# KyleKWKim/LLM-guided-Multimodal-MIL

Measured on AMD Instinct MI355X. Metric: bags/sec fwd+bwd, N=1024 patches D=512, higher is better.
Workload: dtype f32; 1 GPU; 32 bags/GPU x 1024 patches x 512 dims, image-only gated-attention MIL fwd+BCE+bwd+allreduce+Adam (BASELINE config 2; x1 GPUs = 32 bags); bags_per_gpu=32, patches=1024, dim=512, global_bags=32, parallelism=dp1, mode=train (dropout 0.5 on patches + 0.25 before the head, in-kernel masks), accum=1, batches_cycled=4, launch=eager

## Files before the change

### llm-guided-multimodal-mil_amd/csrc/gated_pool.hip

```cpp
#include "mil_common.h"
#include "philox.h"
#include "gate_reduce.h"
#include <type_traits>

#define GF_TM 128
#define GF_BK 32
#define GF_NG 384

typedef __attribute__((address_space(3))) void lds_void;
__device__ __forceinline__ unsigned bitmask1(unsigned m, int b) { return (unsigned)__builtin_amdgcn_sbfe((int)m, b, 1); }
__device__ __forceinline__ float keep_if(float v, unsigned m, int b) {
    return __uint_as_float(__float_as_uint(v) & bitmask1(m, b));
}
template <bool DROP>
__global__ __launch_bounds__(512) void k_gate_fwd(const float* __restrict__ x, const float* __restrict__ Wv,
                                                       const float* __restrict__ bv, const float* __restrict__ Wu,
                                                       const float* __restrict__ bu, const float* __restrict__ wvec,
                                                       const float* __restrict__ battn, float* __restrict__ scores,
                                                       float* __restrict__ gates, int R, int L,
                                                       const uint32_t* __restrict__ xbits, float xscale) {
    __shared__ __attribute__((aligned(16))) float smem[2 * (GF_TM + GF_NG) * 32];
    float* xs = smem;
    float* ws = smem + 2 * GF_TM * 32;
    const int tid = threadIdx.x, lane = tid & 63, wave = tid >> 6;
// ... 1253 lines not shown
    auto xwrite = [&](int i, int buf) {
        f32x4 v = __builtin_bit_cast(f32x4, rx[i]);
        if (DROP) {
            const unsigned mm = rm[i] >> (4 * (xc4 & 7));
#pragma unroll
            for (int e = 0; e < 4; ++e) v[e] = keep_if(v[e], mm, e);
        }
        *reinterpret_cast<f32x4*>(xw + (buf * GB_BKR + 8 * i) * 128) = v;
    };
    auto awrite_v = [&](int i, int buf) {
        const f32x4 v = __builtin_bit_cast(f32x4, rv[i]);
        const f32x4 a = (rds[i] * w4) * __builtin_bit_cast(f32x4, ru[i]);
        const f32x4 t = a * v;
        rt[i] = t;
        *reinterpret_cast<f32x4*>(aw + (buf * GB_BKR + 16 * i) * 128) = a - t * v;
    };
    auto awrite_u = [&](int i, int buf, bool pub) {
        const f32x4 t = rt[i], u = __builtin_bit_cast(f32x4, ru[i]);
        const f32x4 pu = t - t * u;
        *reinterpret_cast<f32x4*>(aw + (buf * GB_BKR + 16 * i) * 128 + 32) = pu;
        if (pub) {
            const f32x4 v = __builtin_bit_cast(f32x4, rv[i]);
            acc_bv += (rds[i] * w4) * u - t * v;
            acc_bu += pu;
            acc_w += (rds[i] * v) * u;
            if (ad4 == 0) acc_ds += rds[i];
        }
    };

    f32x16 acc[2][2];
#pragma unroll
    for (int a = 0; a < 2; ++a)
#pragma unroll
        for (int b = 0; b < 2; ++b)
#pragma unroll
            for (int i = 0; i < 16; ++i) acc[a][b][i] = 0.f;

#pragma unroll
    for (int i = 0; i < 4; ++i) xload(i, rbeg);
#pragma unroll
    for (int i = 0; i < 2; ++i) aload(i, rbeg);
#pragma unroll
    for (int i = 0; i < 4; ++i) xwrite(i, 0);
#pragma unroll
    for (int i = 0; i < 2; ++i) { awrite_v(i, 0); awrite_u(i, 0, jt == 0); }
#pragma unroll
    for (int i = 0; i < 4; ++i) xload(i, rbeg + GB_BKR);
#pragma unroll
    for (int i = 0; i < 2; ++i) aload(i, rbeg + GB_BKR);
    __syncthreads();

    auto slice = [&](int sl, auto buf_c) {
        constexpr int buf = decltype(buf_c)::value;
        const int row2 = rbeg + (sl + 2) * GB_BKR;
        const bool pub = ((sl + 1) % NJ) == jt;
        const float* apb = ap + buf * GB_BKR * 128;
        const float* bpb = bp + buf * GB_BKR * 128;
        float fa[2][2], fb[2][2];
        fa[0][0] = apb[0]; fa[0][1] = apb[64]; fb[0][0] = bpb[0]; fb[0][1] = bpb[64];
#pragma unroll
        for (int ks = 0; ks < GB_BKR / 2; ++ks) {
            const int q = ks & 1;
            acc[0][0] = __builtin_amdgcn_mfma_f32_32x32x2f32(fa[q][0], fb[q][0], acc[0][0], 0, 0, 0);
            __builtin_amdgcn_sched_barrier(0);
            if (ks + 1 < GB_BKR / 2) {
                fa[q ^ 1][0] = apb[(ks + 1) * 256]; fa[q ^ 1][1] = apb[(ks + 1) * 256 + 64];
                fb[q ^ 1][0] = bpb[(ks + 1) * 256]; fb[q ^ 1][1] = bpb[(ks + 1) * 256 + 64];
            }
            __builtin_amdgcn_sched_barrier(0);
            acc[0][1] = __builtin_amdgcn_mfma_f32_32x32x2f32(fa[q][0], fb[q][1], acc[0][1], 0, 0, 0);
            __builtin_amdgcn_sched_barrier(0);
            if (ks >= 1 && ks <= 4) xwrite(ks - 1, buf ^ 1);
            if (ks == 5) awrite_v(0, buf ^ 1);
            if (ks == 6) awrite_u(0, buf ^ 1, pub);
            if (ks == 7) awrite_v(1, buf ^ 1);
            if (ks == 8) awrite_u(1, buf ^ 1, pub);
            __builtin_amdgcn_sched_barrier(0);
            acc[1][0] = __builtin_amdgcn_mfma_f32_32x32x2f32(fa[q][1], fb[q][0], acc[1][0], 0, 0, 0);
            __builtin_amdgcn_sched_barrier(0);
            if (ks >= 1 && ks <= 4) xload(ks - 1, row2);
            if (ks == 6) aload(0, row2);
            if (ks == 8) aload(1, row2);
            __builtin_amdgcn_sched_barrier(0);
            acc[1][1] = __builtin_amdgcn_mfma_f32_32x32x2f32(fa[q][1], fb[q][1], acc[1][1], 0, 0, 0);
            __builtin_amdgcn_sched_barrier(0);
        }
    };
    int sl = 0;
    for (; sl + 1 < nloop; sl += 2) {
        slice(sl, std::integral_constant<int, 0>{});
        __syncthreads();
        slice(sl + 1, std::integral_constant<int, 1>{});
        __syncthreads();
    }
    if (sl < nloop) {
        slice(sl, std::integral_constant<int, 0>{});
        __syncthreads();
    }

    {
        float* tw = smem + wave * (64 * 64);
#pragma unroll
        for (int a = 0; a < 2; ++a)
#pragma unroll
            for (int b = 0; b < 2; ++b)
#pragma unroll
                for (int i = 0; i < 16; ++i) tw[(32 * a + mfma32_row(i, h)) * 64 + 32 * b + r] = acc[a][b][i];
        __syncthreads();
        float* pt = part + ((size_t)s * GF_NG + 128 * m + 64 * wi) * L + j0 + 64 * wj;
        const int c4 = lane & 15, rr = lane >> 4;
        const float* t0 = smem_all + wave * (64 * 64);
        const float* t1 = smem_all + (2 * 2 * GB_BKR * 128) + wave * (64 * 64);
#pragma unroll
        for (int pass = 0; pass < 8; ++pass) {
            const int row = 4 * (pass + 8 * grp) + rr;
            const f32x4 v = *reinterpret_cast<const f32x4*>(t0 + row * 64 + 4 * c4) +
                            *reinterpret_cast<const f32x4*>(t1 + row * 64 + 4 * c4);
            *reinterpret_cast<f32x4*>(pt + (size_t)row * L + 4 * c4) = v;
        }
    }

    {
        float* redf = smem_all;
        const int arow_all = arow + 16 * grp;
        __syncthreads();
#pragma unroll
        for (int e = 0; e < 4; ++e) {
            redf[(arow_all * 3 + 0) * 64 + 4 * ad4 + e] = acc_bv[e];
            redf[(arow_all * 3 + 1) * 64 + 4 * ad4 + e] = acc_bu[e];
            redf[(arow_all * 3 + 2) * 64 + 4 * ad4 + e] = acc_w[e];
        }
        __syncthreads();
        float* pb = pbias + ((size_t)s * NJ + jt) * 4 * 192;
        if (threadIdx.x < 192) {
            const int which = threadIdx.x / 64, d = threadIdx.x % 64;
            float v = 0.f;
#pragma unroll
            for (int g = 0; g < 32; ++g) v += redf[(g * 3 + which) * 64 + d];
            pb[which * 192 + 64 * m + d] = v;
        }
        if (m == 0) {
            __syncthreads();
            redf[threadIdx.x] = acc_ds;
            __syncthreads();
            if (threadIdx.x == 0) {
                float v = 0.f;
                for (int g = 0; g < 512; g += 16) v += redf[g];
                pb[3 * 192] = v;
            }
        }
    }
}

#include "gate_reduce.h"

static inline int split_kg(int R, int L) {
#if defined(GB_NO_KG2)
    return 1;
#endif
    const int NJ = L / 128;
    const int smax = (MIL_NUM_CU) / (3 * NJ);
    return (smax >= 1 && R / smax >= 512) ? 2 : 1;
}
static inline int split_plan(int R, int L, int* KC_out) {
    const int NJ = L / 128;
    int smax = (2 * MIL_NUM_CU / split_kg(R, L)) / (3 * NJ);
    if (smax < 1) smax = 1;
    int kc = ((R + smax - 1) / smax + GB_BKR - 1) / GB_BKR * GB_BKR;
    if (kc < GB_BKR) kc = GB_BKR;
    *KC_out = kc;
    return (R + kc - 1) / kc;
}

extern "C" int mil_abi_version(void) { return 7; }

#define GS_TM 32
#define GS_LS 36
#define GS_THREADS 768
template <bool DROP, int RT>
__global__ __launch_bounds__(GS_THREADS) void k_gate_fwd_r32(const float* __restrict__ x, const float* __restrict__ Wv,
                                                             const float* __restrict__ bv, const float* __restrict__ Wu,
                                                             const float* __restrict__ bu, const float* __restrict__ wvec,
                                                             const float* __restrict__ battn, float* __restrict__ scores,
                                                             float* __restrict__ gates, int R, int L,
                                                             const uint32_t* __restrict__ xbits, float xscale,
                                                             const int32_t* __restrict__ rows_dev) {
    constexpr int TM = GS_TM * RT;
    if (rows_dev != nullptr && (int)(blockIdx.x * TM) >= __builtin_amdgcn_readfirstlane(rows_dev[0])) return;
    __shared__ __attribute__((aligned(16))) float smem[2 * (TM + GF_NG) * GS_LS];
    float* xs = smem;
    float* ws = smem + 2 * TM * GS_LS;
    const int tid = threadIdx.x, lane = tid & 63, wave = tid >> 6;
    const int c = wave >> 1, isu = wave & 1;
    const int r = lane & 31, h = lane >> 5;
    const int row0 = blockIdx.x * TM;
    const float* wsrc[4];
    int wdst[4];
#pragma unroll
    for (int i = 0; i < 4; ++i) {
        const int id = tid + GS_THREADS * i, wrow = id >> 3, ch = id & 7;
        wsrc[i] = (wrow < 192 ? Wv + (size_t)wrow * L : Wu + (size_t)(wrow - 192) * L) + 4 * ch;
        wdst[i] = wrow * GS_LS + 4 * ch;
    }
    const int xrow = (tid % (256 * RT)) >> 3, xch = tid & 7;
    const float* xsrc = x + (size_t)min(row0 + xrow, R - 1) * L + 4 * xch;
    const uint32_t* msrc = DROP ? xbits + (size_t)min(row0 + xrow, R - 1) * (L / 32) : nullptr;
    const int xdst = xrow * GS_LS + 4 * xch;
    f32x4 wreg[2][4], xreg[2];
    unsigned mreg[2] = {0, 0};
    auto gload = [&](int set, int k0) {
#pragma unroll
        for (int i = 0; i < 4; ++i) wreg[set][i] = *reinterpret_cast<const f32x4*>(wsrc[i] + k0);
        xreg[set] = *reinterpret_cast<const f32x4*>(xsrc + k0);
        if (DROP) mreg[set] = msrc[k0 >> 5];
    };
    auto swrite = [&](int set, int buf) {
#pragma unroll
        for (int i = 0; i < 4; ++i) *reinterpret_cast<f32x4*>(ws + buf * GF_NG * GS_LS + wdst[i]) = wreg[set][i];
        if (tid < 256 * RT) {
            f32x4 v = xreg[set];
            if (DROP) {
                const unsigned m = mreg[set] >> (4 * xch);
#pragma unroll
                for (int e = 0; e < 4; ++e) v[e] = keep_if(v[e], m, e) * xscale;
            }
            *reinterpret_cast<f32x4*>(xs + buf * TM * GS_LS + xdst) = v;
        }
    };
    f32x16 acc[RT];
#pragma unroll
    for (int q = 0; q < RT; ++q)
#pragma unroll
        for (int i = 0; i < 16; ++i) acc[q][i] = 0.f;
    const int nslice = L / GF_BK;
    gload(0, 0);
    swrite(0, 0);
    gload(1, min(1, nslice - 1) * GF_BK);
    gload(0, min(2, nslice - 1) * GF_BK);
    __syncthreads();
    auto iteration = [&](int s, int set) {
        const int buf = s & 1;
        const float* xa = xs + buf * TM * GS_LS + r * GS_LS + 4 * h;
        const float* wb = ws + buf * GF_NG * GS_LS + (192 * isu + 32 * c + r) * GS_LS + 4 * h;
        f32x4 fa[RT][4], fb[4];
#pragma unroll
        for (int t = 0; t < 4; ++t) {
#pragma unroll
            for (int q = 0; q < RT; ++q) fa[q][t] = *reinterpret_cast<const f32x4*>(xa + q * GS_TM * GS_LS + 8 * t);
            fb[t] = *reinterpret_cast<const f32x4*>(wb + 8 * t);
        }
        swrite(set, buf ^ 1);
        gload(set, min(s + 3, nslice - 1) * GF_BK);
        __builtin_amdgcn_sched_barrier(0);
#pragma unroll
        for (int t = 0; t < 4; ++t)
#pragma unroll
            for (int jj = 0; jj < 4; ++jj)
#pragma unroll
                for (int q = 0; q < RT; ++q) acc[q] = __builtin_amdgcn_mfma_f32_32x32x2f32(fa[q][t][jj], fb[t][jj], acc[q], 0, 0, 0);
        __syncthreads();
    };
    for (int s = 0; s < nslice; s += 2) {
        iteration(s, 1);
        if (s + 1 < nslice) iteration(s + 1, 0);
    }
    const int d = 32 * c + r;
    float* uex = smem;
    float* sred = smem + 6 * 32 * 33;
#pragma unroll
    for (int q = 0; q < RT; ++q) {
        float gv[16];
        if (q > 0) __syncthreads();
        if (isu) {
            const float bud = bu[d];
#pragma unroll
            for (int i = 0; i < 16; ++i) {
                gv[i] = fast_sigmoid(acc[q][i] + bud);
                uex[(c * 32 + mfma32_row(i, h)) * 33 + r] = gv[i];
            }
        } else {
            const float bvd = bv[d];
#pragma unroll
            for (int i = 0; i < 16; ++i) gv[i] = fast_tanh(acc[q][i] + bvd);
        }
        if (gates != nullptr) {
#pragma unroll
            for (int i = 0; i < 16; ++i) {
                const int gr = row0 + GS_TM * q + mfma32_row(i, h);
                if (gr < R) gates[(size_t)gr * GF_NG + 192 * isu + d] = gv[i];
            }
        }
        __syncthreads();
        if (!isu) {
            const float wd = wvec[d];
#pragma unroll
            for (int i = 0; i < 16; ++i) {
                const int lr = mfma32_row(i, h);
                const float part = half_allsum(wd * gv[i] * uex[(c * 32 + lr) * 33 + r]);
                if (r == 0) sred[c * GS_TM + lr] = part;
            }
        }
        __syncthreads();
        if (tid < GS_TM && row0 + GS_TM * q + tid < R) {
            float sc = battn[0];
#pragma unroll
            for (int cc = 0; cc < 6; ++cc) sc += sred[cc * GS_TM + tid];
            scores[row0 + GS_TM * q + tid] = sc;
// ... 198 lines not shown
        g.offset_dev = offset_dev;
        return gate_scores_fwd_impl(x, Wv, bv, Wu, bu, w, b, scores, gates, R, L, MIL_GATE_D, nullptr, xscale, &g, stream, nullptr,
                                    nullptr, rows_dev, tmap, Wp);
    }
    return gate_scores_fwd_impl(x, Wv, bv, Wu, bu, w, b, scores, gates, R, L, MIL_GATE_D, xbits, xscale, nullptr, stream, nullptr,
                                nullptr, rows_dev, tmap, Wp);
}

int gate_fwd_with_pool(const float* x, const float* Wv, const float* bv, const float* Wu, const float* bu, const float* w,
                       const float* b, float* scores, float* gates, int R, int L, int draw, uint32_t* xbits, float xscale,
                       uint32_t* mbits, float mscale, int B, uint64_t seed, uint64_t mseed, uint64_t offset,
                       const int32_t* offset_dev, const int32_t* tile_map, int T, float* partials, const float* Wf, float* hrow,
                       int* fused, void* stream, const uint16_t* Wp) {
    GateFwdPool pl{};
    pl.tile_map = tile_map;
    pl.partials = partials;
    pl.T = T;
    pl.Wf = Wf;
    pl.hrow = hrow;
    pl.mbits = draw ? nullptr : mbits;
    pl.mscale = mscale;
    if (draw) {
        if (!xbits || !mbits || (L % 64) != 0 || B <= 0) return MIL_EINVAL;
        GateFwdGen g{};
        g.xbits_out = xbits;
        g.mbits_out = mbits;
        g.B = B;
        g.seed_lo = (uint32_t)seed;
        g.seed_hi = (uint32_t)(seed >> 32);
        g.mseed_lo = (uint32_t)mseed;
        g.mseed_hi = (uint32_t)(mseed >> 32);
        g.offset = offset;
        g.offset_dev = offset_dev;
        return gate_scores_fwd_impl(x, Wv, bv, Wu, bu, w, b, scores, gates, R, L, MIL_GATE_D, nullptr, xscale, &g, stream, &pl, fused,
                                    nullptr, nullptr, Wp);
    }
    return gate_scores_fwd_impl(x, Wv, bv, Wu, bu, w, b, scores, gates, R, L, MIL_GATE_D, xbits, xscale, nullptr, stream, &pl, fused,
                                nullptr, nullptr, Wp);
}

static int launch_pool_partial(const float* x, const float* scores, const int32_t* tile_map, int T, int L,
                               float* partials, const float* Wf, int C, float* hrow, hipStream_t st,
                               const uint32_t* xbits = nullptr, float xscale = 1.0f, const uint32_t* mbits = nullptr,
                               float mscale = 1.0f) {
    if (T <= 0) return MIL_OK;
    const bool nt = (size_t)T * MIL_POOL_TILE * L * sizeof(float) > MIL_STREAM_BYTES;
#define POOL_LAUNCH(NQ_) do { \
        if (nt) hipLaunchKernelGGL((k_pool_partial<NQ_, true>), dim3(T), dim3(256), 0, st, x, scores, tile_map, partials, L, Wf, C, hrow, xbits, xscale, mbits, mscale); \
        else hipLaunchKernelGGL((k_pool_partial<NQ_, false>), dim3(T), dim3(256), 0, st, x, scores, tile_map, partials, L, Wf, C, hrow, xbits, xscale, mbits, mscale); } while (0)
    switch (L / 256) {
        case 1: POOL_LAUNCH(1); break;
        case 2: POOL_LAUNCH(2); break;
        case 3: POOL_LAUNCH(3); break;
        default: POOL_LAUNCH(4); break;
    }
#undef POOL_LAUNCH
    MIL_CHECK_LAUNCH();
    return MIL_OK;
}

__global__ __launch_bounds__(256) void k_build_tile_map(const int32_t* __restrict__ bag_len, int B, int32_t* __restrict__ tile_map,
                                                        int32_t* __restrict__ bag_tile_off, int32_t* __restrict__ rows_out,
                                                        int T_cap) {
    build_tile_map_block(bag_len, B, tile_map, bag_tile_off, rows_out, T_cap);
}

extern "C" int mil_build_tile_map(const int32_t* bag_len, int B, int32_t* tile_map, int32_t* bag_tile_off, int32_t* rows_out,
                                  int T_cap, void* stream) {
    if (!bag_len || !tile_map || !bag_tile_off || !rows_out || B <= 0 || B > 1024 || T_cap < 0) return MIL_EINVAL;
    hipLaunchKernelGGL(k_build_tile_map, dim3(1), dim3(256), 0, (hipStream_t)stream, bag_len, B, tile_map, bag_tile_off, rows_out,
                       T_cap);
    MIL_CHECK_LAUNCH();
    return MIL_OK;
}

extern "C" int mil_attn_pool_partial_h(const float* x, const float* scores, const int32_t* tile_map, int T, int L,
                                       float* partials, const float* Wf, int C, float* hrow, const uint32_t* xbits,
                                       float xscale, const uint32_t* mbits, float mscale, void* stream) {
    if (!x || !scores || !tile_map || !partials || !Wf || !hrow) return MIL_EINVAL;
    if (L <= 0 || (L % 256) != 0 || L > 1024 || T < 0 || C <= 0 || C > 4) return MIL_EINVAL;
    return launch_pool_partial(x, scores, tile_map, T, L, partials, Wf, C, hrow, (hipStream_t)stream, xbits, xscale, mbits,
                               mscale);
}

extern "C" int mil_attn_pool_bwd_from_h(const float* scores, const float* lse, const float* hrow, const float* dz,
                                        const float* cdot, const int32_t* tile_map, int T, int C, float* ds, void* stream) {
    if (!scores || !lse || !hrow || !dz || !cdot || !tile_map || !ds || T < 0 || C <= 0 || C > 4) return MIL_EINVAL;
    if (T == 0) return MIL_OK;
    hipLaunchKernelGGL(k_pool_ds_from_h, dim3((T + 7) / 8), dim3(256), 0, (hipStream_t)stream, scores, lse, hrow, dz, cdot,
                       tile_map, T, C, ds);
    MIL_CHECK_LAUNCH();
    return MIL_OK;
}

extern "C" int mil_attn_pool_partial(const float* x, const float* scores, const int32_t* tile_map, int T, int L,
                                     float* partials, const uint32_t* xbits, float xscale, void* stream) {
    if (!x || !scores || !tile_map || !partials) return MIL_EINVAL;
    if (L <= 0 || (L % 256) != 0 || L > 1024 || T < 0) return MIL_EINVAL;
    return launch_pool_partial(x, scores, tile_map, T, L, partials, nullptr, 0, nullptr, (hipStream_t)stream, xbits, xscale);
}

extern "C" int mil_attn_pool_fwd(const float* x, const float* scores, const int32_t* tile_map,
                                 const int32_t* bag_tile_off, int T, int B, int L, float* partials, float* M,
                                 float* lse, const uint32_t* xbits, float xscale, void* stream) {
    if (!x || !scores || !tile_map || !bag_tile_off || !partials || !M || !lse) return MIL_EINVAL;
    if (L <= 0 || (L % 256) != 0 || L > 1024 || B < 0 || T < 0) return MIL_EINVAL;
    hipStream_t st = (hipStream_t)stream;
    const int rc = launch_pool_partial(x, scores, tile_map, T, L, partials, nullptr, 0, nullptr, st, xbits, xscale);
    if (rc != MIL_OK) return rc;
    if (B > 0) {
        hipLaunchKernelGGL(k_pool_merge, dim3(B, L / 128), dim3(256), 0, st, partials, bag_tile_off, M, lse, L, T);
        MIL_CHECK_LAUNCH();
    }
    return MIL_OK;
}

extern "C" int mil_attn_pool_bwd(const float* x, const float* scores, const float* lse, const float* dM,
                                 const float* cdot, const int32_t* tile_map, int T, int L, float* ds, float* dx,
                                 const uint32_t* xbits, float xscale, void* stream) {
    if (!x || !scores || !lse || !dM || !cdot || !tile_map || !ds) return MIL_EINVAL;
    if (L <= 0 || (L % 256) != 0 || L > 1024 || T < 0) return MIL_EINVAL;
    if (T == 0) return MIL_OK;
    hipStream_t st = (hipStream_t)stream;
    switch (L / 256) {
        case 1: hipLaunchKernelGGL(k_pool_bwd_ds<1>, dim3(T), dim3(256), 0, st, x, scores, lse, dM, cdot, tile_map, ds, dx, L, xbits, xscale); break;
        case 2: hipLaunchKernelGGL(k_pool_bwd_ds<2>, dim3(T), dim3(256), 0, st, x, scores, lse, dM, cdot, tile_map, ds, dx, L, xbits, xscale); break;
        case 3: hipLaunchKernelGGL(k_pool_bwd_ds<3>, dim3(T), dim3(256), 0, st, x, scores, lse, dM, cdot, tile_map, ds, dx, L, xbits, xscale); break;
        default: hipLaunchKernelGGL(k_pool_bwd_ds<4>, dim3(T), dim3(256), 0, st, x, scores, lse, dM, cdot, tile_map, ds, dx, L, xbits, xscale); break;
    }
    MIL_CHECK_LAUNCH();
    return MIL_OK;
}

template <bool XB16>
static void launch_gate_bwd_dw(const void* x, const float* gates, const float* ds, const float* w, float* part, float* pbias,
                               int R, int L, int kc, int NJ, int S, const uint32_t* xbits, hipStream_t st,
                               const int32_t* rows_dev = nullptr) {
    const dim3 grid(S * 3 * NJ);
    if (split_kg(R, L) == 2) {
        if (xbits) hipLaunchKernelGGL((k_gate_bwd_dw<XB16, 2, true>), grid, dim3(512), 0, st, x, gates, ds, w, part, pbias, R, L, kc, NJ, xbits, rows_dev);
        else hipLaunchKernelGGL((k_gate_bwd_dw<XB16, 2, false>), grid, dim3(512), 0, st, x, gates, ds, w, part, pbias, R, L, kc, NJ, xbits, rows_dev);
    } else {
        if (xbits) hipLaunchKernelGGL((k_gate_bwd_dw<XB16, 1, true>), grid, dim3(256), 0, st, x, gates, ds, w, part, pbias, R, L, kc, NJ, xbits, rows_dev);
        else hipLaunchKernelGGL((k_gate_bwd_dw<XB16, 1, false>), grid, dim3(256), 0, st, x, gates, ds, w, part, pbias, R, L, kc, NJ, xbits, rows_dev);
    }
}

static inline bool use_dw2(int R, int L) {
#if defined(GB_NO_DW2)
    return false;
#endif
    return split_kg(R, L) == 2 && (long long)R * L < (1ll << 29);
}
static inline size_t gate_bwd_ws_floats(int S, int L) { return (size_t)S * GF_NG * L + (size_t)S * (L / 128) * 4 * 192; }

extern "C" size_t mil_gate_bwd_workspace_floats(int R, int L) {
    if (R <= 0 || L <= 0 || (L % 128) != 0) return 0;
    int kc;
    const int S = split_plan(R, L, &kc);
    return gate_bwd_ws_floats(S, L);
}

static int gate_bwd_partials_impl(const float* x, const float* gates, const float* ds, const float* w, int R, int L,
                                  int D, float* workspace, size_t workspace_floats, const uint32_t* xbits,
                                  const int32_t* rows_dev, void* stream) {
    if (!x || !gates || !ds || !w || !workspace) return MIL_EINVAL;
    if (D != MIL_GATE_D || L <= 0 || (L % 128) != 0 || R <= 0) return MIL_EINVAL;
    int kc;
    const int S = split_plan(R, L, &kc);
    if (workspace_floats < gate_bwd_ws_floats(S, L)) return MIL_ENOSPC;
    const int NJ = L / 128;
    if (use_dw2(R, L)) {
        float* pb = workspace + (size_t)S * GF_NG * L;
        if (xbits)
            hipLaunchKernelGGL(k_gate_bwd_dw2<true>, dim3(S * 3 * NJ), dim3(512), 0, (hipStream_t)stream, x, gates, ds, w, workspace, pb,
                               R, L, kc, NJ, xbits, rows_dev);
        else
            hipLaunchKernelGGL(k_gate_bwd_dw2<false>, dim3(S * 3 * NJ), dim3(512), 0, (hipStream_t)stream, x, gates, ds, w, workspace, pb,
                               R, L, kc, NJ, xbits, rows_dev);
        MIL_CHECK_LAUNCH();
        return MIL_OK;
    }
    launch_gate_bwd_dw<false>((const void*)x, gates, ds, w, workspace, workspace + (size_t)S * GF_NG * L, R, L, kc, NJ, S, xbits,
                              (hipStream_t)stream, rows_dev);
    MIL_CHECK_LAUNCH();
    return MIL_OK;
}

extern "C" int mil_gate_bwd_partials(const float* x, const float* gates, const float* ds, const float* w, int R, int L,
                                     int D, float* workspace, size_t workspace_floats, const uint32_t* xbits,
                                     void* stream) {
    return gate_bwd_partials_impl(x, gates, ds, w, R, L, D, workspace, workspace_floats, xbits, nullptr, stream);
}
extern "C" int mil_gate_bwd_partials_rows(const float* x, const float* gates, const float* ds, const float* w, int R, int L,
                                          int D, float* workspace, size_t workspace_floats, const uint32_t* xbits,
                                          const int32_t* rows_dev, void* stream) {
    return gate_bwd_partials_impl(x, gates, ds, w, R, L, D, workspace, workspace_floats, xbits, rows_dev, stream);
}

extern "C" int mil_gate_bwd_reduce(const float* workspace, int R, int L, float* dWv, float* dbv, float* dWu, float* dbu,
                                   float* dw, float* db, int accumulate, float xscale, void* stream) {
    if (!workspace || !dWv || !dbv || !dWu || !dbu || !dw || !db) return MIL_EINVAL;
    if (L <= 0 || (L % 128) != 0 || R <= 0) return MIL_EINVAL;
    int kc;
    const int S = split_plan(R, L, &kc);
    const int nthreads = GF_NG * (L / 4) + GR_NB * (3 * 192 + 1);
    hipLaunchKernelGGL(k_gate_bwd_reduce, dim3((nthreads + 255) / 256), dim3(256), 0, (hipStream_t)stream, workspace,
                       workspace + (size_t)S * GF_NG * L, S, use_dw2(R, L) ? S * (L / 128) : S, L, dWv, dbv, dWu, dbu, dw, db,
                       accumulate, xscale);
    MIL_CHECK_LAUNCH();
    return MIL_OK;
}

extern "C" int mil_gate_bwd_params_head(const float* x, const float* gates, const float* ds, const float* w, int R, int L,
                                        int D, float* workspace, size_t workspace_floats, float* dWv, float* dbv,
                                        float* dWu, float* dbu, float* dw, float* db, int accumulate, const float* dz,
                                        const float* M, float* dWf, float* dbf, int B, int C, const float* loss_bag,
                                        float* loss_out, const uint32_t* xbits, float xscale, void* stream) {
    if (!dWv || !dbv || !dWu || !dbu || !dw || !db || !dz || !M || !dWf || !dbf) return MIL_EINVAL;
    if (B <= 0 || C <= 0 || C > 32 || (loss_bag && !loss_out)) return MIL_EINVAL;
    const int rc = mil_gate_bwd_partials(x, gates, ds, w, R, L, D, workspace, workspace_floats, xbits, stream);
    if (rc != MIL_OK) return rc;
    int kc;
    const int S = split_plan(R, L, &kc);
    const int nthreads = GF_NG * (L / 4) + GR_NB * (3 * 192 + 1);
    const int nred = (nthreads + 255) / 256, nhead = C * ((L + 63) / 64) + 1;
    const HeadBwdArgs head{dz, M, dWf, dbf, loss_bag, loss_out, B, L, C, accumulate};
    hipLaunchKernelGGL(k_gate_bwd_reduce, dim3(nred + nhead), dim3(256), 0, (hipStream_t)stream, workspace,
                       workspace + (size_t)S * GF_NG * L, S, use_dw2(R, L) ? S * (L / 128) : S, L, dWv, dbv, dWu, dbu, dw, db,
                       accumulate, xbits ? xscale : 1.0f, nred, head);
    MIL_CHECK_LAUNCH();
    return MIL_OK;
}

extern "C" int mil_gate_bwd_reduce_head(const float* workspace, int R, int L, float* dWv, float* dbv, float* dWu, float* dbu,
                                        float* dw, float* db, int accumulate, float xscale, const float* dz, const float* M,
                                        float* dWf, float* dbf, int B, int C, const float* loss_bag, float* loss_out,
                                        void* stream) {
    if (!workspace || !dWv || !dbv || !dWu || !dbu || !dw || !db || !dz || !M || !dWf || !dbf) return MIL_EINVAL;
    if (L <= 0 || (L % 128) != 0 || R <= 0 || B <= 0 || C <= 0 || C > 32 || (loss_bag && !loss_out)) return MIL_EINVAL;
    int kc;
    const int S = split_plan(R, L, &kc);
    const int nthreads = GF_NG * (L / 4) + GR_NB * (3 * 192 + 1);
    const int nred = (nthreads + 255) / 256, nhead = C * ((L + 63) / 64) + 1;
    const HeadBwdArgs head{dz, M, dWf, dbf, loss_bag, loss_out, B, L, C, accumulate};
    hipLaunchKernelGGL(k_gate_bwd_reduce, dim3(nred + nhead), dim3(256), 0, (hipStream_t)stream, workspace,
                       workspace + (size_t)S * GF_NG * L, S, use_dw2(R, L) ? S * (L / 128) : S, L, dWv, dbv, dWu, dbu, dw, db,
                       accumulate, xscale, nred, head);
    MIL_CHECK_LAUNCH();
    return MIL_OK;
}

int gate_bwd_reduce_head_adam_impl(const float* workspace, int R, int L, float* dWv, float* dbv, float* dWu, float* dbu,
                                   float* dw, float* db, int accumulate, float xscale, const float* dz, const float* M,
                                   float* dWf, float* dbf, int B, int C, const float* loss_bag, float* loss_out,
                                   float* param_flat, const float* grad_flat, size_t n_param, float* exp_avg,
                                   float* exp_avg_sq, int step, const int* step_dev, float lr, const float* lr_dev, float beta1,
                                   float beta2, float eps, float weight_decay, float grad_scale, void* stream, int* done = nullptr,
                                   uint16_t* Wp = nullptr);

extern "C" int mil_gate_bwd_reduce_head_adam(const float* workspace, int R, int L, float* dWv, float* dbv, float* dWu,
                                             float* dbu, float* dw, float* db, int accumulate, float xscale, const float* dz,
                                             const float* M, float* dWf, float* dbf, int B, int C, const float* loss_bag,
                                             float* loss_out, float* param_flat, const float* grad_flat, size_t n_param,
                                             float* exp_avg, float* exp_avg_sq, int step, float lr, float beta1, float beta2,
                                             float eps, float weight_decay, float grad_scale, void* stream) {
    return gate_bwd_reduce_head_adam_impl(workspace, R, L, dWv, dbv, dWu, dbu, dw, db, accumulate, xscale, dz, M, dWf, dbf, B, C,
                                          loss_bag, loss_out, param_flat, grad_flat, n_param, exp_avg, exp_avg_sq, step, nullptr,
                                          lr, nullptr, beta1, beta2, eps, weight_decay, grad_scale, stream);
}

int gate_bwd_reduce_head_adam_impl(const float* workspace, int R, int L, float* dWv, float* dbv, float* dWu, float* dbu,
                                   float* dw, float* db, int accumulate, float xscale, const float* dz, const float* M,
                                   float* dWf, float* dbf, int B, int C, const float* loss_bag, float* loss_out,
                                   float* param_flat, const float* grad_flat, size_t n_param, float* exp_avg,
                                   float* exp_avg_sq, int step, const int* step_dev, float lr, const float* lr_dev, float beta1,
                                   float beta2, float eps, float weight_decay, float grad_scale, void* stream, int* done,
                                   uint16_t* Wp) {
    if (!workspace || !dWv || !dbv || !dWu || !dbu || !dw || !db || !dz || !M || !dWf || !dbf) return MIL_EINVAL;
    if (!param_flat || !grad_flat || !exp_avg || !exp_avg_sq || (step_dev == nullptr && step < 1)) return MIL_EINVAL;
    if (step_dev != nullptr) step = 1;
    if (L <= 0 || (L % 128) != 0 || R <= 0 || B <= 0 || C <= 0 || C > 32 || (loss_bag && !loss_out)) return MIL_EINVAL;
    const float* outs[8] = {dWv, dbv, dWu, dbu, dw, db, dWf, dbf};
    const size_t lens[8] = {(size_t)192 * L, 192, (size_t)192 * L, 192, 192, 1, (size_t)C * L, (size_t)C};
    for (int i = 0; i < 8; ++i)
        if (outs[i] < grad_flat || outs[i] + lens[i] > grad_flat + n_param) return MIL_EINVAL;
    if (((dWv - grad_flat) | (dWu - grad_flat)) & 3) return MIL_EINVAL;
    if ((reinterpret_cast<uintptr_t>(param_flat) | reinterpret_cast<uintptr_t>(grad_flat) | reinterpret_cast<uintptr_t>(exp_avg) |
         reinterpret_cast<uintptr_t>(exp_avg_sq)) & 15)
        return MIL_EINVAL;
    int kc;
    const int S = split_plan(R, L, &kc);
    const int nthreads = GF_NG * (L / 4) + GR_NB * (3 * 192 + 1);
    const int nred = (nthreads + 255) / 256, nhead = C * ((L + 63) / 64) + 1;
    const HeadBwdArgs head{dz, M, dWf, dbf, loss_bag, loss_out, B, L, C, accumulate};
    const double bc1 = 1.0 - pow((double)beta1, (double)step);
    const double bc2 = 1.0 - pow((double)beta2, (double)step);
    const AdamFuse ad{param_flat, grad_flat, exp_avg, exp_avg_sq, (float)bc1, beta1, beta2, eps, weight_decay, grad_scale,
                      (float)sqrt(bc2), step_dev, lr, lr_dev, step_dev ? done : nullptr};
    hipLaunchKernelGGL(k_gate_bwd_reduce, dim3(nred + nhead), dim3(256), 0, (hipStream_t)stream, workspace,
                       workspace + (size_t)S * GF_NG * L, S, use_dw2(R, L) ? S * (L / 128) : S, L, dWv, dbv, dWu, dbu, dw, db,
                       accumulate, xscale, nred, head, ad, nullptr, nullptr, (unsigned short*)Wp);
    MIL_CHECK_LAUNCH();
    return MIL_OK;
}

__global__ __launch_bounds__(256) void k_gate_pieces(const float* __restrict__ Wv, const float* __restrict__ Wu,
                                                     unsigned short* __restrict__ Wp, int L) {
    const int L4 = L / 4;
    const int idx = blockIdx.x * 256 + threadIdx.x;
    if (idx >= GF_NG * L4) return;
    const int n = idx / L4, k = 4 * (idx % L4);
    const float* src = (n < MIL_GATE_D ? Wv + (size_t)n * L : Wu + (size_t)(n - MIL_GATE_D) * L) + k;
    gp_store4(Wp, n, k, *reinterpret_cast<const f32x4*>(src));
}

extern "C" int mil_gate_pieces(const float* Wv, const float* Wu, uint16_t* Wp, int L, void* stream) {
    if (!Wv || !Wu || !Wp || L <= 0 || (L % 32) != 0) return MIL_EINVAL;
    if ((reinterpret_cast<uintptr_t>(Wv) | reinterpret_cast<uintptr_t>(Wu) | reinterpret_cast<uintptr_t>(Wp)) & 15) return MIL_EINVAL;
    hipLaunchKernelGGL(k_gate_pieces, dim3((GF_NG * (L / 4) + 255) / 256), dim3(256), 0, (hipStream_t)stream, Wv, Wu,
                       (unsigned short*)Wp, L);
    MIL_CHECK_LAUNCH();
    return MIL_OK;
}

extern "C" int mil_gate_bwd_params(const float* x, const float* gates, const float* ds, const float* w, int R, int L,
// ... 290 lines not shown
```

Before: 153,900 bags/s.

## Add split-bf16 MFMA weight-gradient kernel for gated attention backward

Adds a new weight-gradient kernel for the gate backward pass. It splits each f32 operand into three bf16 pieces and accumulates six cross products with 32x32x16 bf16 MFMA, standing in for the previous dW path. It double-buffers LDS staging and interleaves global loads and LDS writes with the MFMA steps. It also remaps block IDs across XCDs and folds the bias and w-vector reductions into the same kernel. The kernel is on by default, with an environment variable to turn it off, and it trades some precision (roughly f32 via 3xbf16) for matrix-core throughput.

```diff
diff --git a/llm-guided-multimodal-mil_amd/csrc/gated_pool.hip b/llm-guided-multimodal-mil_amd/csrc/gated_pool.hip
--- a/llm-guided-multimodal-mil_amd/csrc/gated_pool.hip
+++ b/llm-guided-multimodal-mil_amd/csrc/gated_pool.hip
@@ -1429,7 +1429,249 @@
     }
 }
 
-#include "gate_reduce.h"
+typedef float dwp_f32x2 __attribute__((ext_vector_type(2)));
+typedef __bf16 dwp_bf16x2 __attribute__((ext_vector_type(2)));
+#define DWP_IMG_BYTES (3 * 2 * 128 * 16)
+#define DWP_PIECE_BYTES (2 * 128 * 16)
+
+__device__ __forceinline__ void dwp_split8(const float (&v)[8], u32x4_t (&out)[3]) {
+#pragma unroll
+    for (int i = 0; i < 4; ++i) {
+        const dwp_f32x2 v2 = {v[2 * i], v[2 * i + 1]};
+        const dwp_bf16x2 p0 = __builtin_convertvector(v2, dwp_bf16x2);
+        dwp_f32x2 r1 = v2 - __builtin_convertvector(p0, dwp_f32x2);
+        r1[0] = __builtin_isfinite(r1[0]) ? r1[0] : 0.f;
+        r1[1] = __builtin_isfinite(r1[1]) ? r1[1] : 0.f;
+        const dwp_bf16x2 p1 = __builtin_convertvector(r1, dwp_bf16x2);
+        const dwp_f32x2 r2 = r1 - __builtin_convertvector(p1, dwp_f32x2);
+        const dwp_bf16x2 p2 = __builtin_convertvector(r2, dwp_bf16x2);
+        out[0][i] = __builtin_bit_cast(unsigned, p0);
+        out[1][i] = __builtin_bit_cast(unsigned, p1);
+        out[2][i] = __builtin_bit_cast(unsigned, p2);
+    }
+}
+__device__ __forceinline__ float dwp_keep_lane(float v, uint64_t lanemask) {
+    float o;
+    asm("v_cndmask_b32_e64 %0, 0, %1, %2" : "=v"(o) : "v"(v), "s"(lanemask));
+    return o;
+}
+
+template <bool DROP>
+__global__ __launch_bounds__(512) void k_gate_bwd_dw2p(const float* __restrict__ x, const float* __restrict__ gates,
+                                                       const float* __restrict__ ds, const float* __restrict__ wvec,
+                                                       float* __restrict__ part, float* __restrict__ pbias, int R, int L,
+                                                       int KC, int NJ, const uint32_t* __restrict__ xbits,
+                                                       const int32_t* __restrict__ rows_dev) {
+    __shared__ __attribute__((aligned(16))) float smem_all[2 * 2 * 2 * GB_BKR * 128];
+    if (rows_dev != nullptr) R = min(R, __builtin_amdgcn_readfirstlane(rows_dev[0]));
+    const int grp = __builtin_amdgcn_readfirstlane((int)(threadIdx.x >> 8));
+    float* smem = smem_all + grp * (2 * 2 * GB_BKR * 128);
+    const int tid = threadIdx.x & 255, lane = tid & 63;
+    const int wave = __builtin_amdgcn_readfirstlane(tid >> 6);
+    const int wi = wave >> 1, wj = wave & 1;
+    const int r = lane & 31, h = lane >> 5;
+    int bid = blockIdx.x;
+    {
+        const int nwg = gridDim.x, q = nwg >> 3, rem = nwg & 7, xcd = bid & 7;
+        bid = (xcd < rem ? xcd * (q + 1) : rem * (q + 1) + (xcd - rem) * q) + (bid >> 3);
+    }
+    const int jt = bid % NJ, m = (bid / NJ) % 3, s = bid / (3 * NJ);
+    const int j0 = jt * 128;
+    const int cbeg = min(s * KC, R), cend = min(R, cbeg + KC);
+    const int half = ((cend - cbeg + 2 * GB_BKR - 1) / (2 * GB_BKR)) * GB_BKR;
+    const int rbeg = min(cend, cbeg + grp * half), rend = min(cend, rbeg + half);
+    const int nloop = (min(half, cend - cbeg) + 15) / 16;
+
+    const bool is_u = (wave & 1) != 0;
+    const int skh = wave >> 1;
+    const int sc = 64 * (wave & 1) + lane;
+    const int LW = L >> 5;
+    const int vx = (j0 + sc) * 4, vg = (64 * m + lane) * 4;
+    const int vd = (8 * skh + (lane & 7)) * 4;
+    const float wd = wvec[64 * m + lane];
+    char* const sbase = reinterpret_cast<char*>(smem);
+    char* const swr = sbase + (skh * 128 + sc) * 16;
+    const char* const fa_rd = sbase + h * 2048 + (64 * wi + r) * 16;
+    const char* const fb_rd = sbase + DWP_IMG_BYTES + h * 2048 + (64 * wj + r) * 16;
+
+    float rx[8], rv[8], ru[8], rds = 0.f;
+    uint64_t rm[8] = {0, 0, 0, 0, 0, 0, 0, 0};
+    float acc_b = 0.f, acc_w = 0.f, acc_ds = 0.f;
+
+    auto x_srd = [&](int row) {
+        return __builtin_amdgcn_make_buffer_rsrc((void*)(x + (size_t)row * L), 0, row < rend ? L * 4 : 0, MIL_SRD_FLAGS);
+    };
+    auto g_srd = [&](int row) {
+        return __builtin_amdgcn_make_buffer_rsrc((void*)(gates + (size_t)row * GF_NG), 0, row < rend ? GF_NG * 4 : 0, MIL_SRD_FLAGS);
+    };
+    auto d_srd = [&](int row0) {
+        return __builtin_amdgcn_make_buffer_rsrc((void*)(ds + row0), 0, max(rend - row0, 0) * 4, MIL_SRD_FLAGS);
+    };
+    auto xload = [&](int row0) {
+#pragma unroll
+        for (int j = 0; j < 8; ++j)
+            rx[j] = __uint_as_float(__builtin_amdgcn_raw_buffer_load_b32(x_srd(row0 + 8 * skh + j), vx, 0, 0));
+        if (DROP) {
+            const int wofs = (j0 + 64 * (wave & 1)) >> 5;
+#pragma unroll
+            for (int j = 0; j < 8; ++j) {
+                const int row = max(min(row0 + 8 * skh + j, R - 1), 0);
+                rm[j] = *reinterpret_cast<const uint64_t*>(xbits + (size_t)row * LW + wofs);
+            }
+        }
+    };
+    auto aload = [&](int row0) {
+#pragma unroll
+        for (int j = 0; j < 8; ++j) {
+            const __amdgpu_buffer_rsrc_t g = g_srd(row0 + 8 * skh + j);
+            rv[j] = __uint_as_float(__builtin_amdgcn_raw_buffer_load_b32(g, vg, 0, 0));
+            ru[j] = __uint_as_float(__builtin_amdgcn_raw_buffer_load_b32(g, vg + 192 * 4, 0, 0));
+        }
+        rds = __uint_as_float(__builtin_amdgcn_raw_buffer_load_b32(d_srd(row0), vd, 0, 0));
+    };
+    auto xwrite = [&](int buf) {
+        float v[8];
+#pragma unroll
+        for (int j = 0; j < 8; ++j) v[j] = DROP ? dwp_keep_lane(rx[j], rm[j]) : rx[j];
+        u32x4_t o[3];
+        dwp_split8(v, o);
+        char* dst = swr + buf * (2 * DWP_IMG_BYTES) + DWP_IMG_BYTES;
+#pragma unroll
+        for (int q = 0; q < 3; ++q) *reinterpret_cast<u32x4_t*>(dst + q * DWP_PIECE_BYTES) = o[q];
+    };
+    auto awrite = [&](int buf, bool pub) {
+        float v[8];
+        auto form = [&](auto u_c) {
+            constexpr bool U = decltype(u_c)::value;
+#pragma unroll
+            for (int j = 0; j < 8; ++j) {
+                const float dj = __uint_as_float((unsigned)__builtin_amdgcn_readlane((int)__float_as_uint(rds), j));
+                const float a = (dj * wd) * ru[j];
+                const float t = a * rv[j];
+                v[j] = U ? t - t * ru[j] : a - t * rv[j];
+                if (pub) {
+                    acc_b += v[j];
+                    if (!U) {
+                        acc_w += (dj * rv[j]) * ru[j];
+                        acc_ds += dj;
+                    }
+                }
+            }
+        };
+        if (is_u) form(std::true_type{});
+        else form(std::false_type{});
+        u32x4_t o[3];
+        dwp_split8(v, o);
+        char* dst = swr + buf * (2 * DWP_IMG_BYTES);
+#pragma unroll
+        for (int q = 0; q < 3; ++q) *reinterpret_cast<u32x4_t*>(dst + q * DWP_PIECE_BYTES) = o[q];
+    };
+
+    f32x16 acc[2][2];
+#pragma unroll
+    for (int a = 0; a < 2; ++a)
+#pragma unroll
+        for (int b = 0; b < 2; ++b)
+#pragma unroll
+            for (int i = 0; i < 16; ++i) acc[a][b][i] = 0.f;
+
+    int nextpub = jt;
+    xload(rbeg);
+    aload(rbeg);
+    xwrite(0);
+    awrite(0, nextpub == 0);
+    if (nextpub == 0) nextpub += NJ;
+    xload(rbeg + 16);
+    aload(rbeg + 16);
+    __syncthreads();
+
+    auto slice = [&](int sl, auto buf_c) {
+        constexpr int buf = decltype(buf_c)::value;
+        const int row2 = rbeg + (sl + 2) * 16;
+        const bool pub = (sl + 1) == nextpub;
+        if (pub) nextpub += NJ;
+        const char* ab = fa_rd + buf * (2 * DWP_IMG_BYTES);
+        const char* bb = fb_rd + buf * (2 * DWP_IMG_BYTES);
+        u32x4_t fa[3][2], fb[3][2];
+        auto rd = [&](const char* p, int q, int t) { return *reinterpret_cast<const u32x4_t*>(p + q * DWP_PIECE_BYTES + t * 512); };
+        fa[0][0] = rd(ab, 0, 0); fa[0][1] = rd(ab, 0, 1); fb[2][0] = rd(bb, 2, 0); fb[2][1] = rd(bb, 2, 1);
+        fa[1][0] = rd(ab, 1, 0); fa[1][1] = rd(ab, 1, 1); fb[1][0] = rd(bb, 1, 0); fb[1][1] = rd(bb, 1, 1);
+        fa[2][0] = rd(ab, 2, 0); fa[2][1] = rd(ab, 2, 1); fb[0][0] = rd(bb, 0, 0); fb[0][1] = rd(bb, 0, 1);
+        constexpr int TP[6] = {0, 1, 2, 0, 1, 0}, TQ[6] = {2, 1, 0, 1, 0, 0};
+#pragma unroll
+        for (int t = 0; t < 6; ++t) {
+#pragma unroll
+            for (int a = 0; a < 2; ++a)
+#pragma unroll
+                for (int b = 0; b < 2; ++b)
+                    acc[a][b] = __builtin_amdgcn_mfma_f32_32x32x16_bf16(__builtin_bit_cast(gp_bf16x8, fa[TP[t]][a]),
+                                                                        __builtin_bit_cast(gp_bf16x8, fb[TQ[t]][b]), acc[a][b], 0, 0, 0);
+            __builtin_amdgcn_sched_barrier(0);
+            if (t == 0) xwrite(buf ^ 1);
+            if (t == 1) xload(row2);
+            if (t == 2) awrite(buf ^ 1, pub);
+            if (t == 3) aload(row2);
+            __builtin_amdgcn_sched_barrier(0);
+        }
+    };
+    int sl = 0;
+    for (; sl + 1 < nloop; sl += 2) {
+        slice(sl, std::integral_constant<int, 0>{});
+        __syncthreads();
+        slice(sl + 1, std::integral_constant<int, 1>{});
+        __syncthreads();
+    }
+    if (sl < nloop) {
+        slice(sl, std::integral_constant<int, 0>{});
+        __syncthreads();
+    }
+
+    {
+        float* tw = smem + wave * (64 * 64);
+#pragma unroll
+        for (int a = 0; a < 2; ++a)
+#pragma unroll
+            for (int b = 0; b < 2; ++b)
+#pragma unroll
+                for (int i = 0; i < 16; ++i) tw[(32 * a + mfma32_row(i, h)) * 64 + 32 * b + r] = acc[a][b][i];
+        __syncthreads();
+        float* pt = part + ((size_t)s * GF_NG + 128 * m + 64 * wi) * L + j0 + 64 * wj;
+        const int c4 = lane & 15, rr = lane >> 4;
+        const float* t0 = smem_all + wave * (64 * 64);
+        const float* t1 = smem_all + (2 * 2 * GB_BKR * 128) + wave * (64 * 64);
+#pragma unroll
+        for (int pass = 0; pass < 8; ++pass) {
+            const int row = 4 * (pass + 8 * grp) + rr;
+            const f32x4 v = *reinterpret_cast<const f32x4*>(t0 + row * 64 + 4 * c4) +
+                            *reinterpret_cast<const f32x4*>(t1 + row * 64 + 4 * c4);
+            *reinterpret_cast<f32x4*>(pt + (size_t)row * L + 4 * c4) = v;
+        }
+    }
+
+    {
+        float* redf = smem_all;
+        const int g4 = grp * 2 + skh;
+        __syncthreads();
+        if (is_u) {
+            redf[(g4 * 3 + 1) * 64 + lane] = acc_b;
+        } else {
+            redf[(g4 * 3 + 0) * 64 + lane] = acc_b;
+            redf[(g4 * 3 + 2) * 64 + lane] = acc_w;
+            if (lane == 0) redf[4 * 3 * 64 + g4] = acc_ds;
+        }
+        __syncthreads();
+        float* pb = pbias + ((size_t)s * NJ + jt) * 4 * 192;
+        if (threadIdx.x < 192) {
+            const int which = threadIdx.x / 64, d = threadIdx.x % 64;
+            float v = 0.f;
+#pragma unroll
+            for (int g = 0; g < 4; ++g) v += redf[(g * 3 + which) * 64 + d];
+            pb[which * 192 + 64 * m + d] = v;
+        } else if (threadIdx.x == 192 && m == 0) {
+            pb[3 * 192] = (redf[768] + redf[769]) + (redf[770] + redf[771]);
+        }
+    }
+}
 
 static inline int split_kg(int R, int L) {
 #if defined(GB_NO_KG2)
@@ -1934,6 +2176,10 @@
 #endif
     return split_kg(R, L) == 2 && (long long)R * L < (1ll << 29);
 }
+static inline bool dw_pieces_enabled() {
+    const char* e = getenv("MIL_DW_PIECES");
+    return e == nullptr || e[0] != '0';
+}
 static inline size_t gate_bwd_ws_floats(int S, int L) { return (size_t)S * GF_NG * L + (size_t)S * (L / 128) * 4 * 192; }
 
 extern "C" size_t mil_gate_bwd_workspace_floats(int R, int L) {
@@ -1954,6 +2200,16 @@
     const int NJ = L / 128;
     if (use_dw2(R, L)) {
         float* pb = workspace + (size_t)S * GF_NG * L;
+        if (dw_pieces_enabled()) {
+            if (xbits)
+                hipLaunchKernelGGL(k_gate_bwd_dw2p<true>, dim3(S * 3 * NJ), dim3(512), 0, (hipStream_t)stream, x, gates, ds, w, workspace, pb,
+                                   R, L, kc, NJ, xbits, rows_dev);
+            else
+                hipLaunchKernelGGL(k_gate_bwd_dw2p<false>, dim3(S * 3 * NJ), dim3(512), 0, (hipStream_t)stream, x, gates, ds, w, workspace, pb,
+                                   R, L, kc, NJ, xbits, rows_dev);
+            MIL_CHECK_LAUNCH();
+            return MIL_OK;
+        }
         if (xbits)
             hipLaunchKernelGGL(k_gate_bwd_dw2<true>, dim3(S * 3 * NJ), dim3(512), 0, (hipStream_t)stream, x, gates, ds, w, workspace, pb,
                                R, L, kc, NJ, xbits, rows_dev);
```

Result: slower. 148,200 bags/s, median of 2 (-3.7%).
